# VITA-Group/Open-L2O

Measured on NVIDIA H100. Metric: coordinate-updates/sec (N_params x unroll_steps), higher is better.
Workload: dtype f32

## Files before the change

open_l2o_b200/csrc/cwlstm_tc.cuh:

```cuda
#pragma once
#include "cwlstm_common.cuh"

namespace l2o {
namespace tc {

constexpr int kH = 20;
constexpr int kN = 4 * kH;
constexpr int kTile = 64;
constexpr int kU = 5;
constexpr int kFwdWG = 3;
constexpr int kFwdThreads = 128 * kFwdWG;
template <int N>
struct IC {
  static constexpr int value = N;
};

template <class C>
struct Geo {
  static constexpr bool FC = C::FC;
  static constexpr int ColH1 = FC ? 24 : 4, ColH2 = FC ? 44 : 24;
  static constexpr int ColOne = FC ? 20 : C::F;
  static constexpr int KB = FC ? 8 : 6;
  static constexpr int L1Lo = 0, L1Hi = FC ? 6 : 3;
  static constexpr int L2Lo = FC ? 2 : 0, L2Hi = KB;
  static constexpr int K1 = 8 * (L1Hi - L1Lo), K2 = 8 * (L2Hi - L2Lo);
  static constexpr int N1 = FC ? 48 : 24, N2 = 48;
  static constexpr int B1Floats = K1 * kN, B2Floats = K2 * kN, T1Floats = kN * N1, T2Floats = kN * N2;
  static constexpr int FwdFloats = 2 * (B1Floats + B2Floats);
  static constexpr int AllFloats = FwdFloats + 2 * (T1Floats + T2Floats);
  static_assert(!FC || C::F == 20, "fc preprocessing: dim 20");
  static_assert(FC || C::F <= 3, "feature chunk: at most 3 features");
};
constexpr int kImgMaxFloats = Geo<Cfg<L2O_PRE_FC, 2, 20, 20, 20>>::AllFloats;

__device__ __forceinline__ uint32_t smem_u32(const void* p) { return (uint32_t)__cvta_generic_to_shared(p); }

__device__ __forceinline__ void mbar_init(uint64_t* bar, uint32_t count) {
  asm volatile("mbarrier.init.shared::cta.b64 [%0], %1;" ::"r"(smem_u32(bar)), "r"(count));
}
__device__ __forceinline__ void mbar_expect_tx(uint64_t* bar, uint32_t bytes) {
  asm volatile("mbarrier.arrive.expect_tx.shared::cta.b64 _, [%0], %1;" ::"r"(smem_u32(bar)), "r"(bytes) : "memory");
}
__device__ __forceinline__ void mbar_wait(uint64_t* bar, uint32_t parity) {
  asm volatile(
      "{\n\t"
      ".reg .pred p;\n\t"
      "WAIT_LOOP:\n\t"
      "mbarrier.try_wait.parity.shared::cta.b64 p, [%0], %1;\n\t"
      "@p bra WAIT_DONE;\n\t"
      "bra WAIT_LOOP;\n\t"
      "WAIT_DONE:\n\t"
      "}\n" ::"r"(smem_u32(bar)),
      "r"(parity)
      : "memory");
}
__device__ __forceinline__ void fence_barrier_init() { asm volatile("fence.mbarrier_init.release.cluster;" ::: "memory"); }
__device__ __forceinline__ void fence_proxy_async() { asm volatile("fence.proxy.async.shared::cta;" ::: "memory"); }
__device__ __forceinline__ void tma_bulk_g2s(void* dst, const void* src, uint32_t bytes, uint64_t* bar) {
  asm volatile("cp.async.bulk.shared::cluster.global.mbarrier::complete_tx::bytes [%0], [%1], %2, [%3];" ::"r"(
                   smem_u32(dst)),
               "l"(src), "r"(bytes), "r"(smem_u32(bar))
               : "memory");
}
__device__ __forceinline__ void stage_image(float* dst, const float* src, uint32_t bytes, uint64_t* bar) {
  if (threadIdx.x == 0) {
    mbar_expect_tx(bar, bytes);
    tma_bulk_g2s(dst, src, bytes, bar);
  }
  mbar_wait(bar, 0);
}

__device__ __forceinline__ void wg_fence() { asm volatile("wgmma.fence.sync.aligned;" ::: "memory"); }
__device__ __forceinline__ void wg_commit() { asm volatile("wgmma.commit_group.sync.aligned;" ::: "memory"); }
template <int N>
__device__ __forceinline__ void wg_wait() {
  asm volatile("wgmma.wait_group.sync.aligned %0;" ::"n"(N) : "memory");
}

__device__ __forceinline__ uint64_t make_desc(uint32_t saddr, uint32_t lbo, uint32_t sbo) {
  return (uint64_t)((saddr & 0x3FFFFu) >> 4) | ((uint64_t)(lbo >> 4) << 16) | ((uint64_t)(sbo >> 4) << 32);
}
__device__ __forceinline__ uint64_t img_desc(const float* p, int ncols) {
  return make_desc(smem_u32(p), (uint32_t)(ncols / 8) * 128u, 128u);
}
__host__ __device__ constexpr uint64_t img_kstep(int ncols) { return (uint64_t)((2 * (ncols / 8) * 128) >> 4); }

#define L2O_ACC8(b) "+f"(d[b]), "+f"(d[b + 1]), "+f"(d[b + 2]), "+f"(d[b + 3]), "+f"(d[b + 4]), "+f"(d[b + 5]), \
                    "+f"(d[b + 6]), "+f"(d[b + 7])
__device__ __forceinline__ void mma_rs_n80(float* d, const uint32_t* a, uint64_t b, uint32_t acc) {
  asm volatile(
      "{\n\t.reg .pred p;\n\tsetp.ne.b32 p, %45, 0;\n\t"
      "wgmma.mma_async.sync.aligned.m64n80k8.f32.tf32.tf32 "
      "{%0,%1,%2,%3,%4,%5,%6,%7,%8,%9,%10,%11,%12,%13,%14,%15,%16,%17,%18,%19,"
      "%20,%21,%22,%23,%24,%25,%26,%27,%28,%29,%30,%31,%32,%33,%34,%35,%36,%37,%38,%39}, "
      "{%40,%41,%42,%43}, %44, p, 1, 1;\n\t}\n"
      : L2O_ACC8(0), L2O_ACC8(8), L2O_ACC8(16), L2O_ACC8(24), L2O_ACC8(32)
      : "r"(a[0]), "r"(a[1]), "r"(a[2]), "r"(a[3]), "l"(b), "r"(acc));
}
__device__ __forceinline__ void mma_rs_n48(float* d, const uint32_t* a, uint64_t b, uint32_t acc) {
  asm volatile(
      "{\n\t.reg .pred p;\n\tsetp.ne.b32 p, %29, 0;\n\t"
      "wgmma.mma_async.sync.aligned.m64n48k8.f32.tf32.tf32 "
      "{%0,%1,%2,%3,%4,%5,%6,%7,%8,%9,%10,%11,%12,%13,%14,%15,%16,%17,%18,%19,%20,%21,%22,%23}, "
      "{%24,%25,%26,%27}, %28, p, 1, 1;\n\t}\n"
      : L2O_ACC8(0), L2O_ACC8(8), L2O_ACC8(16)
      : "r"(a[0]), "r"(a[1]), "r"(a[2]), "r"(a[3]), "l"(b), "r"(acc));
}
__device__ __forceinline__ void mma_rs_n24(float* d, const uint32_t* a, uint64_t b, uint32_t acc) {
  asm volatile(
      "{\n\t.reg .pred p;\n\tsetp.ne.b32 p, %17, 0;\n\t"
      "wgmma.mma_async.sync.aligned.m64n24k8.f32.tf32.tf32 "
      "{%0,%1,%2,%3,%4,%5,%6,%7,%8,%9,%10,%11}, "
      "{%12,%13,%14,%15}, %16, p, 1, 1;\n\t}\n"
      : L2O_ACC8(0), "+f"(d[8]), "+f"(d[9]), "+f"(d[10]), "+f"(d[11])
      : "r"(a[0]), "r"(a[1]), "r"(a[2]), "r"(a[3]), "l"(b), "r"(acc));
}
template <int N>
__device__ __forceinline__ void mma_rs(float* d, const uint32_t* a, uint64_t b, uint32_t acc) {
  static_assert(N == 80 || N == 48 || N == 24, "wgmma width");
  if constexpr (N == 80) mma_rs_n80(d, a, b, acc);
  else if constexpr (N == 48) mma_rs_n48(d, a, b, acc);
  else mma_rs_n24(d, a, b, acc);
}

__device__ __forceinline__ float to_tf32(float x) {
  uint32_t r;
  asm("cvt.rna.tf32.f32 %0, %1;" : "=r"(r) : "f"(x));
  return __uint_as_float(r);
}
__device__ __forceinline__ void split_tf32(float x, uint32_t& hi, uint32_t& lo) {
  hi = __float_as_uint(x) & 0xFFFFE000u;
  lo = __float_as_uint(x - __uint_as_float(hi));
}

__host__ __device__ constexpr int vec_unit(int c, int base) { return 5 * ((c - base) & 3) + ((c - base) >> 2); }
__host__ __device__ constexpr int unit_col(int u, int base) { return base + 4 * (u % 5) + u / 5; }
__host__ __device__ constexpr int gate_ref_col(int n) {
  return (2 * ((n >> 3) & 1) + (n & 1)) * kH + 5 * ((n & 7) >> 1) + (n >> 4);
}
__host__ __device__ constexpr int dx_gate_col(int k) { return (k & ~7) + 2 * (k & 3) + ((k >> 2) & 1); }
__host__ __device__ constexpr int dx_group(int c) { return c / 24; }
__host__ __device__ constexpr int dx_unit(int c) {
  return 2 * ((c % 24) >> 3) + (c & 1) >= 5 ? -1 : 5 * ((c & 7) >> 1) + 2 * ((c % 24) >> 3) + (c & 1);
}
__host__ __device__ constexpr int img_index(int k, int n, int ncols) {
  return ((k >> 2) * (ncols / 8) + (n >> 3)) * 32 + (n & 7) * 4 + (k & 3);
}

template <class C>
__device__ __forceinline__ float ext_weight(const float* __restrict__ theta, bool l2, int c, int n) {
  using G = Geo<C>;
  const int col = gate_ref_col(n);
  if (c == G::ColOne) return theta[(l2 ? C::O_B2 : C::O_B1) + col];
  const bool in_h1 = c >= G::ColH1 && c < G::ColH1 + kH, in_h2 = c >= G::ColH2 && c < G::ColH2 + kH;
  if (!l2) {
    if (in_h1) return theta[C::O_W1 + (C::F + vec_unit(c, G::ColH1)) * C::G1 + col];
    if (G::FC && c < kH) return theta[C::O_W1 + vec_unit(c, 0) * C::G1 + col];
    if (!G::FC && c < C::F) return theta[C::O_W1 + c * C::G1 + col];
    return 0.f;
  }
  if (in_h1) return theta[C::O_W2 + vec_unit(c, G::ColH1) * C::G2 + col];
  if (in_h2) return theta[C::O_W2 + (kH + vec_unit(c, G::ColH2)) * C::G2 + col];
  return 0.f;
}
template <class C>
__host__ __device__ constexpr int dx_operand_col(bool l2, int c) {
  using G = Geo<C>;
  return l2 ? unit_col(dx_unit(c), dx_group(c) == 0 ? G::ColH1 : G::ColH2)
            : unit_col(dx_unit(c), dx_group(c) == 0 ? G::ColH1 : 0);
}

template <class C>
__global__ void prep_weights_kernel(const float* __restrict__ theta, float* __restrict__ img, int with_transposed) {
  static_assert(C::H1 == kH && C::H2 == kH && (C::F <= 3 || C::FC), "tc engine: LSTM-20x2, F <= 3 or fc(20)");
  using G = Geo<C>;
  const int nb = (G::K1 + G::K2) * kN;
  const int nt = with_transposed ? kN * (G::N1 + G::N2) : 0;
  for (int e = blockIdx.x * blockDim.x + threadIdx.x; e < nb + nt; e += gridDim.x * blockDim.x) {
    float w;
    float* hi;
    int off, idx;
    if (e < nb) {
      const bool l2 = e >= G::K1 * kN;
      const int ee = l2 ? e - G::K1 * kN : e;
      const int k = ee / kN, n = ee % kN;
      w = ext_weight<C>(theta, l2, 8 * (l2 ? G::L2Lo : G::L1Lo) + k, n);
      hi = img + (l2 ? 2 * G::B1Floats : 0);
      off = l2 ? G::B2Floats : G::B1Floats;
      idx = img_index(k, n, kN);
    } else {
      const int e2 = e - nb;
      const bool l2 = e2 >= kN * G::N1;
      const int nc = l2 ? G::N2 : G::N1;
      const int ee = l2 ? e2 - kN * G::N1 : e2;
      const int k = ee / nc, n = ee % nc;
      w = dx_unit(n) < 0 ? 0.f : ext_weight<C>(theta, l2, dx_operand_col<C>(l2, n), dx_gate_col(k));
      hi = img + G::FwdFloats + (l2 ? 2 * G::T1Floats : 0);
      off = l2 ? G::T2Floats : G::T1Floats;
      idx = img_index(k, n, nc);
    }
    const float h = to_tf32(w);
    hi[idx] = h;
    hi[off + idx] = to_tf32(w - h);
  }
}

template <int KB>
struct Frag {
  uint32_t hi[KB][4], lo[KB][4];
  __device__ __forceinline__ void zero() {
#pragma unroll
    for (int k = 0; k < KB; ++k)
#pragma unroll
      for (int r = 0; r < 4; ++r) { hi[k][r] = 0u; lo[k][r] = 0u; }
  }
  __device__ __forceinline__ void put_at(int c, int rh, float v) {
    split_tf32(v, hi[c / 8][((c / 4) & 1) * 2 + rh], lo[c / 8][((c / 4) & 1) * 2 + rh]);
  }
  __device__ __forceinline__ float get_at(int c, int rh) const {
    return __uint_as_float(hi[c / 8][((c / 4) & 1) * 2 + rh]) + __uint_as_float(lo[c / 8][((c / 4) & 1) * 2 + rh]);
  }
  template <int COL>
  __device__ __forceinline__ void put(int rh, float v) {
    static_assert(COL % 4 == 0 && COL / 8 < KB, "fragment column");
    put_at(COL, rh, v);
  }
  template <int BASE>
  __device__ __forceinline__ void put_vec(int rh, const float* v) {
    static_assert(BASE % 4 == 0 && (BASE + 19) / 8 < KB, "fragment column");
#pragma unroll
    for (int s = 0; s < kU; ++s) put_at(BASE + 4 * s, rh, v[s]);
  }
};

template <int N, int KB, int LO, int HI>
__device__ __forceinline__ void mma3(float* d, const Frag<KB>& f, uint64_t bh, uint64_t bl) {
  constexpr uint64_t step = img_kstep(N);
#pragma unroll
  for (int kb = LO; kb < HI; ++kb) {
    const uint64_t o = (uint64_t)(kb - LO) * step;
    mma_rs<N>(d, f.lo[kb], bh + o, kb > LO ? 1u : 0u);
    mma_rs<N>(d, f.hi[kb], bl + o, 1u);
    mma_rs<N>(d, f.hi[kb], bh + o, 1u);
  }
}

__host__ __device__ constexpr int acc_idx(int s, int g, int rh) { return 4 * (2 * s + (g >> 1)) + 2 * rh + (g & 1); }

constexpr float kLog2e = 1.4426950408889634f;
__device__ __forceinline__ void lstm_point_fwd(float zi, float zj, float zf, float zo, float& c, float& h) {
  const float Ei = ex2_approx(fminf(-kLog2e * zi, 40.f));
  const float Ej = ex2_approx(fminf(-2.f * kLog2e * zj, 40.f));
  const float Qf = 1.0f + ex2_approx(fminf(fmaf(-kLog2e, zf, -kLog2e), 40.f));
  const float Pij = (1.0f + Ei) * (1.0f + Ej);
  const float cn = fmaf(c, Pij, (1.0f - Ej) * Qf) * rcp_approx(Pij * Qf);
  c = cn;
  const float Ec = ex2_approx(fminf(-2.f * kLog2e * cn, 63.f));
  const float Eo = ex2_approx(fminf(-kLog2e * zo, 63.f));
  h = (1.0f - Ec) * rcp_approx((1.0f + Ec) * (1.0f + Eo));
}
__device__ __forceinline__ float elu_fast(float av) {
  const float em = ex2_approx(kLog2e * av) - 1.0f;
  const float ep = av * fmaf(av, fmaf(av, fmaf(av, 1.0f / 24.0f, 1.0f / 6.0f), 0.5f), 1.0f);
  return av > 0.f ? av : (av > -0.0625f ? ep : em);
}

__device__ __forceinline__ void load5(const float* __restrict__ p, int q, float* v) {
#pragma unroll
  for (int s = 0; s < kU; ++s) v[s] = p[5 * q + s];
}
__device__ __forceinline__ void store5(float* __restrict__ p, int q, const float* v) {
#pragma unroll
  for (int s = 0; s < kU; ++s) p[5 * q + s] = v[s];
}
__device__ __forceinline__ float quad_sum(float v) {
  v += __shfl_xor_sync(0xffffffffu, v, 1);
  return v + __shfl_xor_sync(0xffffffffu, v, 2);
}
__device__ __forceinline__ float from_row(float v, int lane, int rh) {
  return __shfl_sync(0xffffffffu, v, (lane & ~3) | rh);
}

struct FwdExtra {
  const int32_t* step_ptr;
  int32_t t_offset;
  float p_fixed;
};

template <class C>
struct SmemF {
  float img[Geo<C>::FwdFloats];
  float wo[kH + 4];
  float win[64];
  uint64_t wbar;
  uint64_t pad;
  double fx[1];
};
template <class C>
__host__ __device__ constexpr size_t adamc_offset(int T) {
  return (sizeof(SmemF<C>) + (size_t)(T + 1) * sizeof(double) + 15) & ~(size_t)15;
}
template <class C>
__host__ __device__ constexpr size_t fwd_smem_bytes(int T) {
  return adamc_offset<C>(T) + (C::FC ? (size_t)T * 2 * sizeof(float) : 0);
}

template <class C>
__global__ void __launch_bounds__(kFwdThreads, 1) unroll_fwd_kernel(l2o_unroll_args a, NetRt rt, const float* __restrict__ img,
                                                                     float* __restrict__ state_out, FwdExtra ex) {
  using G = Geo<C>;
  extern __shared__ __align__(128) unsigned char smem_raw[];
  SmemF<C>& S = *reinterpret_cast<SmemF<C>*>(smem_raw);
  const int T = a.T;
  const int64_t n = a.n;
  const bool in_kernel_opt = a.opt_kind != L2O_OPT_NONE;
  const bool want_fx = in_kernel_opt && a.fx != nullptr;
  const bool adam_mode = C::NIN == 2 && a.m != nullptr;
  float* adamc = reinterpret_cast<float*>(smem_raw + adamc_offset<C>(T));

  if (want_fx)
    for (int t = threadIdx.x; t <= T; t += blockDim.x) S.fx[t] = 0.0;
  if (threadIdx.x < kH) S.wo[threadIdx.x] = a.theta[C::O_WO + threadIdx.x];
  if (threadIdx.x == kH) S.wo[kH] = a.theta[C::O_BO];
  if constexpr (C::FC) {
    static_assert(!C::FC || C::NIN == 2, "fc nets here are RNNprop nets (two inputs)");
    if (threadIdx.x >= 32 && threadIdx.x < 92) S.win[threadIdx.x - 32] = a.theta[C::O_WIN + threadIdx.x - 32];
    if (adam_mode) {
      const int step0 = ex.step_ptr ? *ex.step_ptr + ex.t_offset : a.step0;
      for (int t = threadIdx.x; t < T; t += blockDim.x) {
        const float p = (ex.step_ptr == nullptr && ex.p_fixed > 0.f) ? ex.p_fixed : (float)(step0 + t);
        adamc[2 * t] = 1.0f - powf(a.beta1, p);
        adamc[2 * t + 1] = 1.0f - powf(a.beta2, p);
      }
    }
  }
  if (threadIdx.x == 0) {
    mbar_init(&S.wbar, 1);
    fence_barrier_init();
  }
  __syncthreads();
  stage_image(S.img, img, G::FwdFloats * 4, &S.wbar);

  const int wg = threadIdx.x >> 7, warp = (threadIdx.x >> 5) & 3, lane = threadIdx.x & 31;
  const int g = lane >> 2, q = lane & 3, own = q & 1;
  const uint64_t b1h = img_desc(S.img, kN), b1l = img_desc(S.img + G::B1Floats, kN);
  const uint64_t b2h = img_desc(S.img + 2 * G::B1Floats, kN), b2l = img_desc(S.img + 2 * G::B1Floats + G::B2Floats, kN);
  const int64_t ntiles = (n + kTile - 1) / kTile;
  const int64_t slot = n * C::SF;
  const float bo = S.wo[kH];
  float wo[kU];
#pragma unroll
  for (int s = 0; s < kU; ++s) wo[s] = S.wo[5 * q + s];
  double imit = 0.0;
  float d[kN / 2];
#pragma unroll
  for (int k = 0; k < kN / 2; ++k) d[k] = 0.f;

  for (int64_t tile = (int64_t)blockIdx.x * kFwdWG + wg; tile < ntiles; tile += (int64_t)gridDim.x * kFwdWG) {
    const int64_t r0 = tile * kTile + warp * 16 + g;
    const int64_t row[2] = {r0, r0 + 8};
    const bool act[2] = {row[0] < n, row[1] < n};
    const int64_t io = own ? row[1] : row[0];
    const bool oact = io < n;
    const bool writer = q < 2 && oact;
    Frag<G::KB> A;
    A.zero();
    float c1[2][kU], c2[2][kU];
#pragma unroll
    for (int rh = 0; rh < 2; ++rh) {
      float h1[kU] = {0.f, 0.f, 0.f, 0.f, 0.f}, h2[kU] = {0.f, 0.f, 0.f, 0.f, 0.f};
#pragma unroll
      for (int s = 0; s < kU; ++s) { c1[rh][s] = 0.f; c2[rh][s] = 0.f; }
      if (act[rh]) {
        const int64_t i = row[rh];
        load5(a.state + i * kH, q, h1);
        load5(a.state + (n + i) * kH, q, c1[rh]);
        load5(a.state + 2 * n * kH + i * kH, q, h2);
        load5(a.state + 2 * n * kH + (n + i) * kH, q, c2[rh]);
        if (a.ckpt) {
          store5(a.ckpt + i * kH, q, h1);
          store5(a.ckpt + (n + i) * kH, q, c1[rh]);
          store5(a.ckpt + 2 * n * kH + i * kH, q, h2);
          store5(a.ckpt + 2 * n * kH + (n + i) * kH, q, c2[rh]);
        }
        if (T == 0 && state_out != a.state) {
          store5(state_out + i * kH, q, h1);
          store5(state_out + (n + i) * kH, q, c1[rh]);
          store5(state_out + 2 * n * kH + i * kH, q, h2);
          store5(state_out + 2 * n * kH + (n + i) * kH, q, c2[rh]);
        }
      }
      A.template put_vec<G::ColH1>(rh, h1);
      A.template put_vec<G::ColH2>(rh, h2);
    }
    if constexpr (G::FC) {
      A.template put<G::ColOne>(0, q == 0 ? 1.0f : 0.f);
      A.template put<G::ColOne>(1, q == 0 ? 1.0f : 0.f);
    }
    float x = 0.f, oa = 0.f, ob = 0.f, am = 0.f, av = 0.f;
    if (oact) {
      if (a.x) x = a.x[io];
      if (in_kernel_opt) { oa = a.opt_a[io]; ob = a.opt_b[io]; }
      if (adam_mode) { am = a.m[io]; av = a.v[io]; }
    }

    for (int t = 0; t < T; ++t) {
      float fval = 0.f, raw0 = 0.f, raw1 = 0.f;
      if (oact) {
        if (in_kernel_opt) {
          optimizee_eval(a.opt_kind, x, oa, ob, a.opt_alpha, a.opt_fscale, fval, raw0);
          if (a.g_rec && q < 2) a.g_rec[(int64_t)t * n + io] = raw0;
        } else if (C::NIN == 2 && !adam_mode) {
          raw0 = a.in_seq[((int64_t)t * 2) * n + io];
          raw1 = a.in_seq[((int64_t)t * 2 + 1) * n + io];
        } else {
          raw0 = a.in_seq[(int64_t)t * n + io];
        }
      }
      if constexpr (G::FC) {
        if (adam_mode) {
          const float gg = raw0;
          am = a.beta1 * am + (1.0f - a.beta1) * gg;
          av = a.beta2 * av + (1.0f - a.beta2) * gg * gg;
          const float mh = am / adamc[2 * t], vh = av / adamc[2 * t + 1];
          const float den = sqrtf(vh) + 1e-8f;
          raw0 = mh / den;
          raw1 = gg / den;
        }
        if (writer && a.feat_rec) {
          a.feat_rec[((int64_t)t * 2) * n + io] = raw0;
          a.feat_rec[((int64_t)t * 2 + 1) * n + io] = raw1;
        }
#pragma unroll
        for (int rh = 0; rh < 2; ++rh) {
          const float m0 = from_row(raw0, lane, rh), m1 = from_row(raw1, lane, rh);
          float u[kU];
#pragma unroll
          for (int s = 0; s < kU; ++s) {
            const int j = 5 * q + s;
            u[s] = elu_fast(fmaf(m1, S.win[kH + j], fmaf(m0, S.win[j], S.win[2 * kH + j])));
          }
          A.template put_vec<0>(rh, u);
        }
      } else {
        float f[C::F];
        preprocess<C>(nullptr, rt, raw0, raw1, f);
#pragma unroll
        for (int rh = 0; rh < 2; ++rh) {
          float v = q == C::F ? 1.0f : 0.f;
#pragma unroll
          for (int k = 0; k < C::F; ++k) {
            const float fk = from_row(f[k], lane, rh);
            if (q == k) v = fk;
          }
          A.template put<0>(rh, v);
        }
      }
      if (want_fx) {
        const double ws = warp_sum_d(q < 2 ? (double)fval : 0.0);
        if (lane == 0) atomicAdd(&S.fx[t], ws);
      }
      wg_fence();
      mma3<kN, G::KB, G::L1Lo, G::L1Hi>(d, A, b1h, b1l);
      wg_commit();
      wg_wait<0>();
#pragma unroll
      for (int rh = 0; rh < 2; ++rh) {
        float h[kU];
#pragma unroll
        for (int s = 0; s < kU; ++s)
          lstm_point_fwd(d[acc_idx(s, 0, rh)], d[acc_idx(s, 1, rh)], d[acc_idx(s, 2, rh)], d[acc_idx(s, 3, rh)], c1[rh][s], h[s]);
        A.template put_vec<G::ColH1>(rh, h);
        if (act[rh]) {
          const int64_t i = row[rh];
          if (a.ckpt) {
            float* ck = a.ckpt + (int64_t)(t + 1) * slot;
            store5(ck + i * kH, q, h);
            store5(ck + (n + i) * kH, q, c1[rh]);
          }
          if (t == T - 1) {
            store5(state_out + i * kH, q, h);
            store5(state_out + (n + i) * kH, q, c1[rh]);
          }
        }
      }
      wg_fence();
      mma3<kN, G::KB, G::L2Lo, G::L2Hi>(d, A, b2h, b2l);
      wg_commit();
      wg_wait<0>();
      float y[2];
#pragma unroll
      for (int rh = 0; rh < 2; ++rh) {
        float h[kU];
        float yp = 0.f;
#pragma unroll
        for (int s = 0; s < kU; ++s) {
          lstm_point_fwd(d[acc_idx(s, 0, rh)], d[acc_idx(s, 1, rh)], d[acc_idx(s, 2, rh)], d[acc_idx(s, 3, rh)], c2[rh][s], h[s]);
          yp = fmaf(h[s], wo[s], yp);
        }
        A.template put_vec<G::ColH2>(rh, h);
        y[rh] = quad_sum(yp) + bo;
        if (act[rh]) {
          const int64_t i = row[rh];
          if (a.ckpt) {
            float* ck = a.ckpt + (int64_t)(t + 1) * slot + 2 * n * kH;
            store5(ck + i * kH, q, h);
            store5(ck + (n + i) * kH, q, c2[rh]);
          }
          if (t == T - 1) {
            store5(state_out + 2 * n * kH + i * kH, q, h);
            store5(state_out + 2 * n * kH + (n + i) * kH, q, c2[rh]);
          }
        }
      }
      const float yo = own ? y[1] : y[0];
      const float dl = rt.tanh_output ? tanh_acc(yo) * rt.scale : yo * rt.scale;
      x += dl;
      if (writer) {
        if (a.delta_seq) a.delta_seq[(int64_t)t * n + io] = dl;
        if (a.labels) {
          const float r = a.labels[(int64_t)t * n + io] - dl;
          imit += 0.5 * (double)r * (double)r;
        }
      }
    }
    float fval = 0.f;
    if (writer) {
      if (in_kernel_opt) {
        float gT;
        optimizee_eval(a.opt_kind, x, oa, ob, a.opt_alpha, a.opt_fscale, fval, gT);
        if (a.g_rec) a.g_rec[(int64_t)T * n + io] = gT;
      }
      if (a.x) a.x[io] = x;
      if (adam_mode) { a.m[io] = am; a.v[io] = av; }
    }
    if (want_fx) {
      const double ws = warp_sum_d((double)fval);
      if (lane == 0) atomicAdd(&S.fx[T], ws);
    }
  }
  if (a.labels && a.imit_loss) {
    const double ws = warp_sum_d(imit);
    if (lane == 0) atomicAdd(a.imit_loss, ws / (double)a.n_total);
  }
  __syncthreads();
  if (want_fx)
    for (int t = threadIdx.x; t <= T; t += blockDim.x) atomicAdd(&a.fx[t], S.fx[t]);
}

}

template <class C>
int tc_launch_fwd(const NetRt& rt, const l2o_unroll_args& a, float* img, cudaStream_t st, int sms, float* state_out = nullptr,
                  tc::FwdExtra ex = tc::FwdExtra{nullptr, 0, 0.f}, bool prep = true) {
  if (prep) tc::prep_weights_kernel<C><<<16, 256, 0, st>>>(a.theta, img, 0);
  auto k = tc::unroll_fwd_kernel<C>;
  const size_t smem = tc::fwd_smem_bytes<C>(a.T);
  if (smem > 227 * 1024) return L2O_E_INVALID;
  if (cudaFuncSetAttribute(k, cudaFuncAttributeMaxDynamicSharedMemorySize, (int)smem) != cudaSuccess) return L2O_E_CUDA;
  const int64_t ntiles = (a.n + tc::kTile - 1) / tc::kTile;
  const int64_t ctas = (ntiles + tc::kFwdWG - 1) / tc::kFwdWG;
  const int grid = (int)(ctas < sms ? ctas : sms);
  k<<<grid, tc::kFwdThreads, smem, st>>>(a, rt, img, state_out ? state_out : a.state, ex);
  return cudaGetLastError() == cudaSuccess ? L2O_OK : L2O_E_CUDA;
}

}
```

open_l2o_b200/csrc/cwlstm_tc_bwd.cuh:

```cuda
#pragma once
#include "cwlstm_tc.cuh"

namespace l2o {
namespace tcb {

using namespace tc;

constexpr int kBwdWG = 2;
constexpr int kBwdThreads = 128 * kBwdWG;
constexpr uint32_t kXaLBO = 8 * 128;
constexpr uint32_t kXbLBO = 10 * 128;
constexpr uint32_t kXaBytes = 8 * kXaLBO;
constexpr uint32_t kXbBytes = 8 * kXbLBO;
constexpr int kBlkL1 = 5, kRowOne2 = 63;

__device__ __forceinline__ void split_bf16x2(float v0, float v1, uint32_t& hi, uint32_t& lo) {
  asm("cvt.rn.bf16x2.f32 %0, %1, %2;" : "=r"(hi) : "f"(v1), "f"(v0));
  const float r0 = v0 - __uint_as_float(hi << 16), r1 = v1 - __uint_as_float(hi & 0xFFFF0000u);
  asm("cvt.rn.bf16x2.f32 %0, %1, %2;" : "=r"(lo) : "f"(r1), "f"(r0));
}
__device__ __forceinline__ void stsm_x4_trans(uint32_t sa, uint32_t r0, uint32_t r1, uint32_t r2, uint32_t r3) {
  asm volatile("stmatrix.sync.aligned.m8n8.x4.trans.shared.b16 [%0], {%1, %2, %3, %4};" ::"r"(sa), "r"(r0), "r"(r1),
               "r"(r2), "r"(r3)
               : "memory");
}
__device__ __forceinline__ void mma_ss_bf16_n80(float* d, uint64_t a, uint64_t b) {
  asm volatile(
      "{\n\t.reg .pred p;\n\tsetp.ne.b32 p, %42, 0;\n\t"
      "wgmma.mma_async.sync.aligned.m64n80k16.f32.bf16.bf16 "
      "{%0,%1,%2,%3,%4,%5,%6,%7,%8,%9,%10,%11,%12,%13,%14,%15,%16,%17,%18,%19,"
      "%20,%21,%22,%23,%24,%25,%26,%27,%28,%29,%30,%31,%32,%33,%34,%35,%36,%37,%38,%39}, "
      "%40, %41, p, 1, 1, 0, 0;\n\t}\n"
      : L2O_ACC8(0), L2O_ACC8(8), L2O_ACC8(16), L2O_ACC8(24), L2O_ACC8(32)
      : "l"(a), "l"(b), "r"(1));
}
__device__ __forceinline__ void wg_bar(int wg) { asm volatile("bar.sync %0, 128;" ::"r"(1 + wg) : "memory"); }
__device__ __forceinline__ void prefetch_l2_bulk(const void* p, uint32_t bytes) {
  asm volatile("cp.async.bulk.prefetch.L2.global [%0], %1;" ::"l"(p), "r"(bytes) : "memory");
}
__device__ __forceinline__ void prefetch_l2(const void* p) { asm volatile("prefetch.global.L2 [%0];" ::"l"(p)); }

__device__ __forceinline__ void unit_bwd(float& zi, float& zj, float& zf, float& zo, float cprev, float dh, float& dc, float& hn) {
  const float i = sigmoid_fast(zi), j = tanh_fast(zj), f = sigmoid_fast(zf + 1.0f), o = sigmoid_fast(zo);
  const float cn = fmaf(f, cprev, i * j);
  const float tcn = tanh_fast(cn);
  hn = tcn * o;
  const float dho = dh * o;
  const float dcv = fmaf(dho, fmaf(-tcn, tcn, 1.0f), dc);
  zi = (dcv * j) * fmaf(-i, i, i);
  zj = (dcv * i) * fmaf(-j, j, 1.0f);
  zf = (dcv * cprev) * fmaf(-f, f, f);
  zo = (dho * tcn) * (1.0f - o);
  dc = dcv * f;
}

template <class C, int MODE>
__device__ __forceinline__ int dw_row(int m) {
  const int p = (m & 7) >> 1, slot = 2 * (m >> 3) + (m & 1);
  if (m == kRowOne2) return MODE == 2 ? C::O_B1 : C::O_B2;
  if (slot < 2 * kBlkL1) {
    const int u = 5 * p + slot % kU;
    if (MODE == 2) return C::O_W1 + (slot < kU ? C::F + u : u) * C::G1;
    return C::O_W2 + (slot < kU ? u : kH + u) * C::G2;
  }
  if (MODE == 0) {
    const int s = slot - 2 * kBlkL1;
    if (s < kU) return C::O_W1 + (C::F + 5 * p + s) * C::G1;
    if (p < C::F) return C::O_W1 + p * C::G1;
    if (p == C::F) return C::O_B1;
  }
  return -1;
}

template <class C, int MODE>
struct SmemB {
  float img[Geo<C>::AllFloats];
  float wo[kH + 4];
  float win[64];
  uint64_t wbar, pad;
};
template <class C, int MODE>
__host__ __device__ constexpr uint32_t stage_bytes() {
  return (MODE == 0 ? 4 : 2) * kXaBytes + 2 * kXbBytes;
}
struct alignas(16) CkRing {
  float h[tc::kTile * kH], c2[tc::kTile * kH], c1[tc::kTile * kH];
  uint64_t barh, bar2, bar1;
};
template <class C, int MODE>
__host__ __device__ constexpr size_t bwd_smem_bytes() {
  return ((sizeof(SmemB<C, MODE>) + 1023) & ~(size_t)1023) +
         (size_t)kBwdWG * (stage_bytes<C, MODE>() + (MODE == 0 ? sizeof(CkRing) : 0));
}

template <class C, int MODE>
__global__ void __launch_bounds__(kBwdThreads, 1) unroll_bwd_kernel(l2o_bwd_args a, NetRt rt, const float* __restrict__ img) {
  using G = Geo<C>;
  static_assert(MODE == 0 ? !C::FC : C::FC, "DM nets: one pass; fc nets: two passes");
  static_assert(MODE != 0 || C::F < 3, "the feature chunk leaves quad thread 3's slot of row 63 to layer 2's 1");
  extern __shared__ __align__(1024) unsigned char smem_raw[];
  SmemB<C, MODE>& S = *reinterpret_cast<SmemB<C, MODE>*>(smem_raw);
  const int wg = threadIdx.x >> 7, warp = (threadIdx.x >> 5) & 3, lane = threadIdx.x & 31;
  const int g = lane >> 2, q = lane & 3;
  const uint32_t stage = smem_u32(smem_raw) + (uint32_t)((sizeof(SmemB<C, MODE>) + 1023) & ~(size_t)1023) +
                         (uint32_t)wg * stage_bytes<C, MODE>();
  constexpr uint32_t kXa2 = 0, kXa1 = 2 * kXaBytes;
  constexpr uint32_t kXb = (MODE == 0 ? 4 : 2) * kXaBytes;
  constexpr bool kL2 = MODE != 2, kL1 = MODE != 1;
  constexpr bool kRing = MODE == 0;
  CkRing& R = *reinterpret_cast<CkRing*>(smem_raw + ((sizeof(SmemB<C, MODE>) + 1023) & ~(size_t)1023) +
                                         (size_t)kBwdWG * stage_bytes<C, MODE>() + (size_t)wg * sizeof(CkRing));
  const bool elected = (threadIdx.x & 127) == 0;

  for (uint32_t o = threadIdx.x * 4; o < kBwdWG * stage_bytes<C, MODE>(); o += blockDim.x * 4) {
    const uint32_t ow = o % stage_bytes<C, MODE>();
    const uint32_t v = (ow < kXaBytes && (ow % kXaLBO) >> 4 == (uint32_t)kRowOne2) ? 0x3F803F80u : 0u;
    asm volatile("st.shared.u32 [%0], %1;" ::"r"(stage - (uint32_t)wg * stage_bytes<C, MODE>() + o), "r"(v) : "memory");
  }
  if (threadIdx.x < kH) S.wo[threadIdx.x] = a.theta[C::O_WO + threadIdx.x];
  if constexpr (C::FC) {
    if (threadIdx.x >= 32 && threadIdx.x < 92) S.win[threadIdx.x - 32] = a.theta[C::O_WIN + threadIdx.x - 32];
  }
  if (threadIdx.x == 0) {
    mbar_init(&S.wbar, 1);
    if (!kRing) fence_barrier_init();
  }
  if (kRing && elected) {
    mbar_init(&R.barh, 1);
    mbar_init(&R.bar2, 1);
    mbar_init(&R.bar1, 1);
    fence_barrier_init();
  }
  fence_proxy_async();
  __syncthreads();
  stage_image(S.img, img, G::AllFloats * 4, &S.wbar);

  const uint64_t b1h = img_desc(S.img, kN), b1l = img_desc(S.img + G::B1Floats, kN);
  const uint64_t b2h = img_desc(S.img + 2 * G::B1Floats, kN), b2l = img_desc(S.img + 2 * G::B1Floats + G::B2Floats, kN);
  const float* tbase = S.img + G::FwdFloats;
  const uint64_t t1h = img_desc(tbase, G::N1), t1l = img_desc(tbase + G::T1Floats, G::N1);
  const uint64_t t2h = img_desc(tbase + 2 * G::T1Floats, G::N2), t2l = img_desc(tbase + 2 * G::T1Floats + G::T2Floats, G::N2);
  const uint64_t xbh = make_desc(stage + kXb, kXbLBO, 128), xbl = make_desc(stage + kXb + kXbBytes, kXbLBO, 128);
  const uint64_t xa2h = make_desc(stage + kXa2, kXaLBO, 128), xa2l = make_desc(stage + kXa2 + kXaBytes, kXaLBO, 128);
  const uint64_t xa1h = make_desc(stage + (MODE == 0 ? kXa1 : kXa2), kXaLBO, 128);
  const uint64_t xa1l = make_desc(stage + (MODE == 0 ? kXa1 : kXa2) + kXaBytes, kXaLBO, 128);

  const int T = a.T;
  const int64_t n = a.n, slot = n * C::SF;
  const int64_t ntiles = (n + tc::kTile - 1) / tc::kTile;
  const bool imit = a.labels != nullptr;
  const float inv_nt = imit ? 1.0f / (float)a.n_total : 0.f;
  float wo[kU];
#pragma unroll
  for (int s = 0; s < kU; ++s) wo[s] = S.wo[5 * q + s];
  float acc_wo[kU] = {0.f, 0.f, 0.f, 0.f, 0.f}, acc_bo = 0.f;
  float aw0[kU] = {0.f, 0.f, 0.f, 0.f, 0.f}, aw1[kU] = {0.f, 0.f, 0.f, 0.f, 0.f}, ab[kU] = {0.f, 0.f, 0.f, 0.f, 0.f};
  float dw[kN / 2];
#pragma unroll
  for (int k = 0; k < kN / 2; ++k) dw[k] = 0.f;
  const int kx = warp * 16 + g;
  const int64_t tstride = (int64_t)gridDim.x * kBwdWG;

  auto ck_block = [&](int64_t tl, int t, int blk) {
    return a.ckpt + (int64_t)t * slot + (blk * n + tl * tc::kTile) * kH;
  };
  auto tile_bytes = [&](int64_t tl) {
    const int64_t r = n - tl * tc::kTile;
    return (uint32_t)((r < tc::kTile ? r : tc::kTile) * kH * 4);
  };
  auto arm = [&](uint64_t* bar, float* dst, int64_t tl, int t, int blk) {
    const uint32_t b = tile_bytes(tl);
    mbar_expect_tx(bar, b);
    tma_bulk_g2s(dst, ck_block(tl, t, blk), b, bar);
  };
  auto ring5 = [&](const float* buf, int rh, bool on, float* v) {
    const float* p = buf + (kx + 8 * rh) * kH + 5 * q;
#pragma unroll
    for (int s = 0; s < kU; ++s) v[s] = on ? p[s] : 0.f;
  };
  if constexpr (kRing) {
    const int64_t tile0 = (int64_t)blockIdx.x * kBwdWG + wg;
    if (elected && tile0 < ntiles) {
      arm(&R.barh, R.h, tile0, T - 1, 2);
      arm(&R.bar2, R.c2, tile0, T - 1, 3);
      arm(&R.bar1, R.c1, tile0, T - 1, 1);
    }
  }
  uint32_t ph = 0;

  Frag<G::KB> A;
  const int blk = lane >> 3;
  const uint32_t la = stage + (uint32_t)((2 * warp + (blk & 1)) * (int)kXaLBO + (blk >> 1) * (int)kXaBytes + (lane & 7) * 16);
  const uint32_t lb = stage + kXb + (uint32_t)((2 * warp + (blk & 1)) * (int)kXbLBO + (blk >> 1) * (int)kXbBytes + (lane & 7) * 16);
  auto stage_x = [&](uint32_t buf, int b0, int nb, int c0, int c1) {
    auto val = [&](int i, int rh) { return A.get_at(i < kU ? c0 + 4 * i : c1 + 4 * (i - kU), rh); };
#pragma unroll
    for (int b = 0; b < nb; ++b) {
      uint32_t h0, l0, h1, l1;
      split_bf16x2(val(2 * b, 0), val(2 * b + 1, 0), h0, l0);
      split_bf16x2(val(2 * b, 1), val(2 * b + 1, 1), h1, l1);
      stsm_x4_trans(la + buf + (uint32_t)(b0 + b) * 128, h0, h1, l0, l1);
    }
  };
  auto stage_dz = [&](const float* z) {
#pragma unroll
    for (int j = 0; j < kN / 8; ++j) {
      uint32_t h0, l0, h1, l1;
      split_bf16x2(z[4 * j], z[4 * j + 1], h0, l0);
      split_bf16x2(z[4 * j + 2], z[4 * j + 3], h1, l1);
      stsm_x4_trans(lb + (uint32_t)j * 128, h0, h1, l0, l1);
    }
  };
  auto dx_dw = [&](auto ncols, float* z, float* x, uint64_t th, uint64_t tl, uint64_t xah, uint64_t xal) {
    constexpr int NX = decltype(ncols)::value;
    uint32_t fh[kN / 8][4], fl[kN / 8][4];
#pragma unroll
    for (int j = 0; j < kN / 8; ++j) {
      split_tf32(z[4 * j + 0], fh[j][0], fl[j][0]);
      split_tf32(z[4 * j + 2], fh[j][1], fl[j][1]);
      split_tf32(z[4 * j + 1], fh[j][2], fl[j][2]);
      split_tf32(z[4 * j + 3], fh[j][3], fl[j][3]);
    }
    constexpr uint64_t step = img_kstep(NX);
    wg_fence();
#pragma unroll
    for (int j = 0; j < kN / 8; ++j) {
      mma_rs<NX>(x, fl[j], th + j * step, j > 0 ? 1u : 0u);
      mma_rs<NX>(x, fh[j], tl + j * step, 1u);
      mma_rs<NX>(x, fh[j], th + j * step, 1u);
    }
    wg_commit();
    constexpr uint64_t sa = (2 * kXaLBO) >> 4, sb = (2 * kXbLBO) >> 4;
#pragma unroll
    for (int kk = 0; kk < tc::kTile / 16; ++kk) {
      mma_ss_bf16_n80(dw, xal + kk * sa, xbh + kk * sb);
      mma_ss_bf16_n80(dw, xah + kk * sa, xbl + kk * sb);
      mma_ss_bf16_n80(dw, xah + kk * sa, xbh + kk * sb);
    }
    wg_commit();
    wg_wait<1>();
  };
  auto flush_dw = [&]() {
    wg_wait<0>();
#pragma unroll
    for (int rh = 0; rh < 2; ++rh) {
      const int r = dw_row<C, MODE>(kx + 8 * rh);
#pragma unroll
      for (int j = 0; j < kN / 8; ++j)
#pragma unroll
        for (int e = 0; e < 2; ++e) {
          float& v = dw[4 * j + 2 * rh + e];
          if (r >= 0 && v != 0.f) atomicAdd(&a.dtheta[r + gate_ref_col(8 * j + 2 * q + e)], (double)v);
          v = 0.f;
        }
    }
  };

  for (int64_t tile = (int64_t)blockIdx.x * kBwdWG + wg; tile < ntiles; tile += tstride) {
    const int64_t r0 = tile * tc::kTile + warp * 16 + g;
    const int64_t row[2] = {r0, r0 + 8};
    const bool act[2] = {row[0] < n, row[1] < n};
    float dc2[2][kU], dh2c[2][kU], dc1[2][kU], dh1c[2][kU];
#pragma unroll
    for (int rh = 0; rh < 2; ++rh)
#pragma unroll
      for (int s = 0; s < kU; ++s) { dc2[rh][s] = 0.f; dh2c[rh][s] = 0.f; dc1[rh][s] = 0.f; dh1c[rh][s] = 0.f; }
    float lam[2];
#pragma unroll
    for (int rh = 0; rh < 2; ++rh) lam[rh] = (kL2 && act[rh] && !imit) ? a.g_rec[(int64_t)T * n + row[rh]] : 0.f;
    A.zero();
    A.template put<(G::ColOne & ~3)>(0, q == (G::ColOne & 3) ? 1.0f : 0.f);
    A.template put<(G::ColOne & ~3)>(1, q == (G::ColOne & 3) ? 1.0f : 0.f);

    for (int t = T - 1; t >= 0; --t) {
      const float* ck = a.ckpt + (int64_t)t * slot;
      const int64_t tl_next = t > 0 ? tile : tile + tstride;
      const int t_next = t > 0 ? t - 1 : T - 1;
      float z[kN / 2];
      float dh1n[2][kU];
      if constexpr (kL2) {
        float c2p[2][kU], dy[2];
        if constexpr (kRing) mbar_wait(&R.barh, 0);
#pragma unroll
        for (int rh = 0; rh < 2; ++rh) {
          float h1n[kU] = {0.f, 0.f, 0.f, 0.f, 0.f}, h2p[kU] = {0.f, 0.f, 0.f, 0.f, 0.f};
#pragma unroll
          for (int s = 0; s < kU; ++s) c2p[rh][s] = 0.f;
          float dtanh = 1.0f;
          if (act[rh]) {
            const int64_t i = row[rh];
            if constexpr (kRing) {
              if (t == T - 1) load5(ck + slot + i * kH, q, h1n);
              ring5(R.h, rh, true, h2p);
            } else {
              load5(ck + slot + i * kH, q, h1n);
              load5(ck + 2 * n * kH + i * kH, q, h2p);
              load5(ck + 2 * n * kH + (n + i) * kH, q, c2p[rh]);
            }
            if (imit) lam[rh] = (a.delta_seq[(int64_t)t * n + i] - a.labels[(int64_t)t * n + i]) * inv_nt;
            if (rt.tanh_output) {
              const float th = a.delta_seq[(int64_t)t * n + i] / rt.scale;
              dtanh = fmaf(-th, th, 1.0f);
            }
          }
          dy[rh] = rt.scale * lam[rh] * dtanh;
          if (!kRing || t == T - 1) A.template put_vec<G::ColH1>(rh, h1n);
          A.template put_vec<G::ColH2>(rh, h2p);
        }
        wg_fence();
        mma3<kN, G::KB, G::L2Lo, G::L2Hi>(z, A, b2h, b2l);
        wg_commit();
        wg_wait<0>();
        if constexpr (kRing) {
          mbar_wait(&R.bar2, ph);
#pragma unroll
          for (int rh = 0; rh < 2; ++rh) ring5(R.c2, rh, act[rh], c2p[rh]);
        }
        if (q == 0) acc_bo += dy[0] + dy[1];
#pragma unroll
        for (int rh = 0; rh < 2; ++rh)
#pragma unroll
          for (int s = 0; s < kU; ++s) {
            float hn;
            unit_bwd(z[acc_idx(s, 0, rh)], z[acc_idx(s, 1, rh)], z[acc_idx(s, 2, rh)], z[acc_idx(s, 3, rh)], c2p[rh][s],
                     fmaf(wo[s], dy[rh], dh2c[rh][s]), dc2[rh][s], hn);
            acc_wo[s] = fmaf(hn, dy[rh], acc_wo[s]);
          }
        wg_bar(wg);
        if (kRing && elected) {
          arm(&R.barh, R.h, tile, t, 0);
          if (tl_next < ntiles) arm(&R.bar2, R.c2, tl_next, t_next, 3);
        }
        stage_x(kXa2, 0, kBlkL1, G::ColH1, G::ColH2);
        stage_dz(z);
        fence_proxy_async();
        wg_bar(wg);
        float x2[G::N2 / 2];
        dx_dw(IC<G::N2>{}, z, x2, t2h, t2l, xa2h, xa2l);
#pragma unroll
// ... 172 lines not shown
```

open_l2o_b200/csrc/l2o_tc.cu:

```cuda
#include "cwlstm_ffma.cuh"
#include "cwlstm_tc.cuh"
#include "cwlstm_tc_bwd.cuh"
#include <cstdlib>
#include <mutex>
#include <utility>
#include <vector>
#include "l2o_internal.h"

namespace l2o {
bool tc_supported(int cfg) { return cfg == 0 || cfg == 1 || cfg == 2; }
bool tc_fwd_ok(const l2o_net* h, const l2o_unroll_args& a) {
  if (a.opt_kind == L2O_OPT_QUADRATIC_BATCH) return false;
  if (h->cfg == 2) return true;
  return a.m == nullptr && a.feat_rec == nullptr;
}
static bool tc_auto_env() {
  static const bool on = !(std::getenv("L2O_TC_AUTO") != nullptr && std::getenv("L2O_TC_AUTO")[0] == '0');
  return on;
}
bool tc_auto_default() { return tc_auto_env(); }
bool tc_bwd_auto_default() { return tc_auto_env(); }

namespace {
struct ImgPool {
  std::mutex mu;
  std::vector<std::pair<int, float*>> free_list;
};
ImgPool& img_pool() {
  static ImgPool* p = new ImgPool();
  return *p;
}
}

void tc_release_image(l2o_net* h) {
  if (!h->tc_img) return;
  ImgPool& P = img_pool();
  std::lock_guard<std::mutex> g(P.mu);
  P.free_list.emplace_back(h->tc_img_dev, h->tc_img);
  h->tc_img = nullptr;
}

static int ensure_image(l2o_net* h) {
  int dev = 0;
  L2O_CUDA_TRY(cudaGetDevice(&dev));
  if (h->tc_img == nullptr || h->tc_img_dev != dev) {
    tc_release_image(h);
    {
      ImgPool& P = img_pool();
      std::lock_guard<std::mutex> g(P.mu);
      for (size_t k = 0; k < P.free_list.size(); ++k)
        if (P.free_list[k].first == dev) {
          h->tc_img = P.free_list[k].second;
          P.free_list.erase(P.free_list.begin() + k);
          break;
        }
    }
    if (h->tc_img == nullptr) L2O_CUDA_TRY(cudaMalloc(&h->tc_img, tc::kImgMaxFloats * sizeof(float)));
    h->tc_img_dev = dev;
    h->tc_img_mode = -1;
  }
  return L2O_OK;
}

bool tc_bwd_ok(const l2o_net* h, const l2o_bwd_args& a) {
  const bool mode_ok = a.labels ? (a.delta_seq != nullptr && a.n_total > 0) : a.g_rec != nullptr;
  if (h->cfg == 2 && a.scratch == nullptr) return false;
  if (h->rt.tanh_output && a.delta_seq == nullptr) return false;
  return tc_supported(h->cfg) && mode_ok;
}

int tc_unroll_bwd(l2o_net* h, const l2o_bwd_args& a, cudaStream_t st) {
  if (!tc_bwd_ok(h, a)) return L2O_E_UNSUPPORTED;
  int rc = ensure_image(h);
  if (rc) return rc;
  const int sms = device_sms();
  if (sms <= 0) return L2O_E_CUDA;
  rc = L2O_E_UNSUPPORTED;
  if (h->cfg == 0) rc = tc_launch_bwd<Cfg<L2O_PRE_IDENTITY, 1, 1, 20, 20>>(h->rt, a, h->tc_img, st, sms);
  if (h->cfg == 1) rc = tc_launch_bwd<Cfg<L2O_PRE_LOGSIGN, 1, 2, 20, 20>>(h->rt, a, h->tc_img, st, sms);
  if (h->cfg == 2) rc = tc_launch_bwd<Cfg<L2O_PRE_FC, 2, 20, 20, 20>>(h->rt, a, h->tc_img, st, sms);
  if (rc == L2O_OK) count_launch(h->cfg == 2 ? 3 : 2);
  h->tc_img_mode = 1;
  if (rc == L2O_E_CUDA) return set_cuda_error(cudaGetLastError(), "tc_unroll_bwd launch");
  return rc;
}

bool tc_step_ok(const l2o_net* h, const l2o_step_args& a) {
  if (h->cfg == 2) return a.m != nullptr;
  return tc_supported(h->cfg) && a.m == nullptr && a.in1 == nullptr && a.feat_out == nullptr;
}

int tc_step(l2o_net* h, const l2o_step_args& s, cudaStream_t st) {
  if (!tc_step_ok(h, s)) return L2O_E_UNSUPPORTED;
  int rc = ensure_image(h);
  if (rc) return rc;
  const int sms = device_sms();
  if (sms <= 0) return L2O_E_CUDA;
  l2o_unroll_args a{};
  a.n = s.n;
  a.T = 1;
  a.theta = s.theta;
  a.in_seq = s.in0;
  a.opt_kind = L2O_OPT_NONE;
  a.x = s.x;
  a.state = const_cast<float*>(s.state_in);
  a.delta_seq = s.delta;
  a.m = s.m;
  a.v = s.v;
  a.beta1 = s.beta1;
  a.beta2 = s.beta2;
  a.step0 = 1;
  a.feat_rec = s.feat_out;
  const tc::FwdExtra ex{s.step_ptr, s.t_offset, s.step_ptr ? 0.f : s.p};
  rc = L2O_E_UNSUPPORTED;
  const bool prep = !(s.reuse_weights && h->tc_img_mode == 0);
  if (h->cfg == 0) rc = tc_launch_fwd<Cfg<L2O_PRE_IDENTITY, 1, 1, 20, 20>>(h->rt, a, h->tc_img, st, sms, s.state_out, ex, prep);
  if (h->cfg == 1) rc = tc_launch_fwd<Cfg<L2O_PRE_LOGSIGN, 1, 2, 20, 20>>(h->rt, a, h->tc_img, st, sms, s.state_out, ex, prep);
  if (h->cfg == 2) rc = tc_launch_fwd<Cfg<L2O_PRE_FC, 2, 20, 20, 20>>(h->rt, a, h->tc_img, st, sms, s.state_out, ex, prep);
  if (rc == L2O_OK) count_launch(prep ? 2 : 1);
  h->tc_img_mode = 0;
  if (rc == L2O_E_CUDA) return set_cuda_error(cudaGetLastError(), "tc_step launch");
  return rc;
}

int tc_unroll_fwd(l2o_net* h, const l2o_unroll_args& a, cudaStream_t st) {
  if (!tc_supported(h->cfg) || !tc_fwd_ok(h, a)) return L2O_E_UNSUPPORTED;
  {
    int rc0 = ensure_image(h);
    if (rc0) return rc0;
  }
  const int sms = device_sms();
  if (sms <= 0) return L2O_E_CUDA;
  int rc = L2O_E_UNSUPPORTED;
  if (h->cfg == 0) rc = tc_launch_fwd<Cfg<L2O_PRE_IDENTITY, 1, 1, 20, 20>>(h->rt, a, h->tc_img, st, sms);
  if (h->cfg == 1) rc = tc_launch_fwd<Cfg<L2O_PRE_LOGSIGN, 1, 2, 20, 20>>(h->rt, a, h->tc_img, st, sms);
  if (h->cfg == 2) rc = tc_launch_fwd<Cfg<L2O_PRE_FC, 2, 20, 20, 20>>(h->rt, a, h->tc_img, st, sms);
  if (rc == L2O_OK) count_launch(2);
  h->tc_img_mode = 0;
  if (rc == L2O_E_CUDA) return set_cuda_error(cudaGetLastError(), "tc_unroll_fwd launch");
  return rc;
}
}
```

Baseline: 1.299 billion.

## Stage LSTM state checkpoints in shared memory and write via bulk async copies

Per-lane scattered 5-float stores of hidden/cell state to checkpoints and state_out are replaced. Each warpgroup now stages a tile's h/c rows into double-buffered shared-memory regions, and an elected thread issues cp.async.bulk shared-to-global copies. This is meant to turn many uncoalesced global stores into contiguous bulk transfers that overlap with compute. In exchange it adds shared-memory footprint, a warpgroup barrier and proxy fence per flush, and host-side 16-byte alignment checks that fall back to another path when they fail.

```diff
diff --git a/open_l2o_b200/csrc/cwlstm_tc.cuh b/open_l2o_b200/csrc/cwlstm_tc.cuh
--- a/open_l2o_b200/csrc/cwlstm_tc.cuh
+++ b/open_l2o_b200/csrc/cwlstm_tc.cuh
@@ -62,6 +62,17 @@
                "l"(src), "r"(bytes), "r"(smem_u32(bar))
                : "memory");
 }
+__device__ __forceinline__ void bulk_s2g(float* dst, const float* src, uint32_t bytes) {
+  asm volatile("cp.async.bulk.global.shared::cta.bulk_group [%0], [%1], %2;" ::"l"(dst), "r"(smem_u32(src)), "r"(bytes)
+               : "memory");
+}
+__device__ __forceinline__ void bulk_commit() { asm volatile("cp.async.bulk.commit_group;" ::: "memory"); }
+template <int N>
+__device__ __forceinline__ void bulk_wait_read() {
+  asm volatile("cp.async.bulk.wait_group.read %0;" ::"n"(N) : "memory");
+}
+__device__ __forceinline__ void bulk_wait_all() { asm volatile("cp.async.bulk.wait_group 0;" ::: "memory"); }
+__device__ __forceinline__ void wg_bar(int wg) { asm volatile("bar.sync %0, 128;" ::"r"(1 + wg) : "memory"); }
 __device__ __forceinline__ void stage_image(float* dst, const float* src, uint32_t bytes, uint64_t* bar) {
   if (threadIdx.x == 0) {
     mbar_expect_tx(bar, bytes);
@@ -287,9 +298,14 @@
   float p_fixed;
 };
 
+constexpr int kStRegions = 2;
+constexpr int kStFloats = 2 * kTile * kH;
+static_assert((kStRegions & (kStRegions - 1)) == 0 && kStRegions >= 2, "staging regions: a power of two");
+
 template <class C>
 struct SmemF {
   float img[Geo<C>::FwdFloats];
+  float stg[kFwdWG][kStRegions][kStFloats];
   float wo[kH + 4];
   float win[64];
   uint64_t wbar;
@@ -356,8 +372,37 @@
 #pragma unroll
   for (int k = 0; k < kN / 2; ++k) d[k] = 0.f;
 
+  const bool elected = (threadIdx.x & 127) == 0;
+  const int kx = warp * 16 + g;
+  uint32_t nst = 0;
+  auto stage5 = [&](int blk, int rh, const float* v) {
+    float* p = &S.stg[wg][nst & (kStRegions - 1)][(blk * kTile + kx + 8 * rh) * kH + 5 * q];
+#pragma unroll
+    for (int s = 0; s < kU; ++s) p[s] = v[s];
+  };
+  auto flush = [&](int64_t tl, int hf, float* dst, float* dst2) {
+    fence_proxy_async();
+    if (elected) bulk_wait_read<kStRegions - 2>();
+    wg_bar(wg);
+    if (elected) {
+      const float* src = S.stg[wg][nst & (kStRegions - 1)];
+      const int64_t rb = tl * kTile, off = (2 * hf * n + rb) * kH;
+      const uint32_t bytes = (uint32_t)((n - rb < kTile ? n - rb : kTile) * kH * 4);
+      if (dst) {
+        bulk_s2g(dst + off, src, bytes);
+        bulk_s2g(dst + off + n * kH, src + kTile * kH, bytes);
+      }
+      if (dst2) {
+        bulk_s2g(dst2 + off, src, bytes);
+        bulk_s2g(dst2 + off + n * kH, src + kTile * kH, bytes);
+      }
+      bulk_commit();
+    }
+    ++nst;
+  };
+
   for (int64_t tile = (int64_t)blockIdx.x * kFwdWG + wg; tile < ntiles; tile += (int64_t)gridDim.x * kFwdWG) {
-    const int64_t r0 = tile * kTile + warp * 16 + g;
+    const int64_t r0 = tile * kTile + kx;
     const int64_t row[2] = {r0, r0 + 8};
     const bool act[2] = {row[0] < n, row[1] < n};
     const int64_t io = own ? row[1] : row[0];
@@ -365,33 +410,29 @@
     const bool writer = q < 2 && oact;
     Frag<G::KB> A;
     A.zero();
-    float c1[2][kU], c2[2][kU];
+    float h1[2][kU], c1[2][kU], h2[2][kU], c2[2][kU];
 #pragma unroll
     for (int rh = 0; rh < 2; ++rh) {
-      float h1[kU] = {0.f, 0.f, 0.f, 0.f, 0.f}, h2[kU] = {0.f, 0.f, 0.f, 0.f, 0.f};
-#pragma unroll
-      for (int s = 0; s < kU; ++s) { c1[rh][s] = 0.f; c2[rh][s] = 0.f; }
+#pragma unroll
+      for (int s = 0; s < kU; ++s) { h1[rh][s] = 0.f; c1[rh][s] = 0.f; h2[rh][s] = 0.f; c2[rh][s] = 0.f; }
       if (act[rh]) {
         const int64_t i = row[rh];
-        load5(a.state + i * kH, q, h1);
+        load5(a.state + i * kH, q, h1[rh]);
         load5(a.state + (n + i) * kH, q, c1[rh]);
-        load5(a.state + 2 * n * kH + i * kH, q, h2);
+        load5(a.state + 2 * n * kH + i * kH, q, h2[rh]);
         load5(a.state + 2 * n * kH + (n + i) * kH, q, c2[rh]);
-        if (a.ckpt) {
-          store5(a.ckpt + i * kH, q, h1);
-          store5(a.ckpt + (n + i) * kH, q, c1[rh]);
-          store5(a.ckpt + 2 * n * kH + i * kH, q, h2);
-          store5(a.ckpt + 2 * n * kH + (n + i) * kH, q, c2[rh]);
-        }
-        if (T == 0 && state_out != a.state) {
-          store5(state_out + i * kH, q, h1);
-          store5(state_out + (n + i) * kH, q, c1[rh]);
-          store5(state_out + 2 * n * kH + i * kH, q, h2);
-          store5(state_out + 2 * n * kH + (n + i) * kH, q, c2[rh]);
-        }
-      }
-      A.template put_vec<G::ColH1>(rh, h1);
-      A.template put_vec<G::ColH2>(rh, h2);
+      }
+      A.template put_vec<G::ColH1>(rh, h1[rh]);
+      A.template put_vec<G::ColH2>(rh, h2[rh]);
+    }
+    float* const copy0 = T == 0 && state_out != a.state ? state_out : nullptr;
+    if (a.ckpt || copy0) {
+#pragma unroll
+      for (int rh = 0; rh < 2; ++rh) { stage5(0, rh, h1[rh]); stage5(1, rh, c1[rh]); }
+      flush(tile, 0, a.ckpt, copy0);
+#pragma unroll
+      for (int rh = 0; rh < 2; ++rh) { stage5(0, rh, h2[rh]); stage5(1, rh, c2[rh]); }
+      flush(tile, 1, a.ckpt, copy0);
     }
     if constexpr (G::FC) {
       A.template put<G::ColOne>(0, q == 0 ? 1.0f : 0.f);
@@ -460,6 +501,9 @@
         const double ws = warp_sum_d(q < 2 ? (double)fval : 0.0);
         if (lane == 0) atomicAdd(&S.fx[t], ws);
       }
+      float* const ck = a.ckpt ? a.ckpt + (int64_t)(t + 1) * slot : nullptr;
+      float* const out = t == T - 1 ? state_out : nullptr;
+      const bool stage = ck || out;
       wg_fence();
       mma3<kN, G::KB, G::L1Lo, G::L1Hi>(d, A, b1h, b1l);
       wg_commit();
@@ -471,19 +515,9 @@
         for (int s = 0; s < kU; ++s)
           lstm_point_fwd(d[acc_idx(s, 0, rh)], d[acc_idx(s, 1, rh)], d[acc_idx(s, 2, rh)], d[acc_idx(s, 3, rh)], c1[rh][s], h[s]);
         A.template put_vec<G::ColH1>(rh, h);
-        if (act[rh]) {
-          const int64_t i = row[rh];
-          if (a.ckpt) {
-            float* ck = a.ckpt + (int64_t)(t + 1) * slot;
-            store5(ck + i * kH, q, h);
-            store5(ck + (n + i) * kH, q, c1[rh]);
-          }
-          if (t == T - 1) {
-            store5(state_out + i * kH, q, h);
-            store5(state_out + (n + i) * kH, q, c1[rh]);
-          }
-        }
-      }
+        if (stage) { stage5(0, rh, h); stage5(1, rh, c1[rh]); }
+      }
+      if (stage) flush(tile, 0, ck, out);
       wg_fence();
       mma3<kN, G::KB, G::L2Lo, G::L2Hi>(d, A, b2h, b2l);
       wg_commit();
@@ -500,19 +534,9 @@
         }
         A.template put_vec<G::ColH2>(rh, h);
         y[rh] = quad_sum(yp) + bo;
-        if (act[rh]) {
-          const int64_t i = row[rh];
-          if (a.ckpt) {
-            float* ck = a.ckpt + (int64_t)(t + 1) * slot + 2 * n * kH;
-            store5(ck + i * kH, q, h);
-            store5(ck + (n + i) * kH, q, c2[rh]);
-          }
-          if (t == T - 1) {
-            store5(state_out + 2 * n * kH + i * kH, q, h);
-            store5(state_out + 2 * n * kH + (n + i) * kH, q, c2[rh]);
-          }
-        }
-      }
+        if (stage) { stage5(0, rh, h); stage5(1, rh, c2[rh]); }
+      }
+      if (stage) flush(tile, 1, ck, out);
       const float yo = own ? y[1] : y[0];
       const float dl = rt.tanh_output ? tanh_acc(yo) * rt.scale : yo * rt.scale;
       x += dl;
@@ -539,6 +563,7 @@
       if (lane == 0) atomicAdd(&S.fx[T], ws);
     }
   }
+  if (elected) bulk_wait_all();
   if (a.labels && a.imit_loss) {
     const double ws = warp_sum_d(imit);
     if (lane == 0) atomicAdd(a.imit_loss, ws / (double)a.n_total);
diff --git a/open_l2o_b200/csrc/cwlstm_tc_bwd.cuh b/open_l2o_b200/csrc/cwlstm_tc_bwd.cuh
--- a/open_l2o_b200/csrc/cwlstm_tc_bwd.cuh
+++ b/open_l2o_b200/csrc/cwlstm_tc_bwd.cuh
@@ -34,7 +34,6 @@
       : L2O_ACC8(0), L2O_ACC8(8), L2O_ACC8(16), L2O_ACC8(24), L2O_ACC8(32)
       : "l"(a), "l"(b), "r"(1));
 }
-__device__ __forceinline__ void wg_bar(int wg) { asm volatile("bar.sync %0, 128;" ::"r"(1 + wg) : "memory"); }
 __device__ __forceinline__ void prefetch_l2_bulk(const void* p, uint32_t bytes) {
   asm volatile("cp.async.bulk.prefetch.L2.global [%0], %1;" ::"l"(p), "r"(bytes) : "memory");
 }
diff --git a/open_l2o_b200/csrc/l2o_tc.cu b/open_l2o_b200/csrc/l2o_tc.cu
--- a/open_l2o_b200/csrc/l2o_tc.cu
+++ b/open_l2o_b200/csrc/l2o_tc.cu
@@ -9,7 +9,9 @@
 
 namespace l2o {
 bool tc_supported(int cfg) { return cfg == 0 || cfg == 1 || cfg == 2; }
+static bool aligned16(const void* p) { return (reinterpret_cast<uintptr_t>(p) & 15) == 0; }
 bool tc_fwd_ok(const l2o_net* h, const l2o_unroll_args& a) {
+  if (!aligned16(a.state) || !aligned16(a.ckpt)) return false;
   if (a.opt_kind == L2O_OPT_QUADRATIC_BATCH) return false;
   if (h->cfg == 2) return true;
   return a.m == nullptr && a.feat_rec == nullptr;
@@ -86,6 +88,7 @@
 }
 
 bool tc_step_ok(const l2o_net* h, const l2o_step_args& a) {
+  if (!aligned16(a.state_out)) return false;
   if (h->cfg == 2) return a.m != nullptr;
   return tc_supported(h->cfg) && a.m == nullptr && a.in1 == nullptr && a.feat_out == nullptr;
 }
```

After: 1.322 billion, median of 6. +1.8%, better.
